# casys-kaist/CoVA

Hardware: AMD Instinct MI355X
Metric: compressed-domain frames/sec (BlobNet+bboxcc) at 1080p b=256 (higher is better)
Workload: dtype f16

## Files before the change

### cova_amd/_lib.py

```python
from __future__ import annotations

import ctypes as C
import os

import numpy as np

_HERE = os.path.dirname(os.path.abspath(__file__))
LIB_PATH = os.path.join(_HERE, "libcovahip.so")

OK = 0
MEM_HOST, MEM_DEVICE = 0, 1
AU_DELTA_UNIT, AU_DISCONT, AU_DROPPABLE = 1, 2, 4


class CovahipError(RuntimeError):
    def __init__(self, status: int, where: str, detail: str = ""):
        self.status = status
        try:
            text = lib().covahip_strerror(status).decode()
        except AttributeError:
            text = "error"
        msg = f"{where}: {text} (status {status})"
        if detail:
            msg += f" [{detail}]"
# ... 142 lines not shown
    "covahip_sort_finalize": (C.c_int, [_P, _P, _SZ, C.POINTER(_SZ), _P, _SZ, C.POINTER(_SZ)]),
    "covahip_sort_mark_seen": (C.c_int, [_P, C.c_uint64]),
    "covahip_sort_num_trackers": (C.c_int, [_P, C.POINTER(_SZ)]),
    "covahip_sort_tracker_info": (C.c_int, [_P, _SZ, C.POINTER(C.c_uint64), C.POINTER(C.c_int),
                                            C.POINTER(C.c_uint64), C.POINTER(C.c_uint64), _P]),
    "covahip_sort_tracker_predict": (C.c_int, [_P, _SZ, C.c_uint64, _P]),
    "covahip_sort_tracker_update": (C.c_int, [_P, _SZ, _P]),
    "covahip_linear_assignment": (_SZ, [_P, _SZ, _SZ, _P, _SZ]),
    "covahip_gopfilter_default_cfg": (None, [C.POINTER(GopFilterCfg)]),
    "covahip_gopfilter_new": (C.c_int, [C.POINTER(GopFilterCfg), C.POINTER(_P)]),
    "covahip_gopfilter_free": (None, [_P]),
    "covahip_gopfilter_push_enc": (C.c_int, [_P, C.c_uint64, C.c_uint64, C.c_uint32]),
    "covahip_gopfilter_push_boxes": (C.c_int, [_P, _P, _SZ, C.c_uint64, _P, _SZ, C.POINTER(_SZ)]),
    "covahip_gopfilter_eos": (C.c_int, [_P, _P, _SZ, C.POINTER(_SZ)]),
    "covahip_gopfilter_take_dropped": (C.c_int, [_P, _P, _SZ, C.POINTER(_SZ)]),
    "covahip_gopfilter_take_track_export": (_SZ, [_P, _P, _SZ, C.POINTER(C.c_int)]),
    "covahip_gopfilter_counters": (C.c_int, [_P, C.POINTER(C.c_uint64), C.POINTER(C.c_uint64),
                                             C.POINTER(C.c_uint64)]),
    "covahip_train_default_cfg": (None, [C.POINTER(TrainCfg)]),
    "covahip_train_create": (C.c_int, [_P, C.POINTER(TrainCfg), _P, _SZ, C.POINTER(_P)]),
    "covahip_train_step": (C.c_int, [_P, _P, _P, C.c_int, C.c_float, C.POINTER(C.c_float), C.c_int]),
    "covahip_train_metrics": (C.c_int, [_P, C.POINTER(C.c_int64)]),
    "covahip_train_weights": (C.c_int, [_P, _P, _SZ, C.POINTER(_SZ)]),
    "covahip_train_grads": (C.c_int, [_P, _P, _SZ]),
    "covahip_train_create_set": (C.c_int, [_P, C.POINTER(TrainCfg), C.c_int, _P, _P, _P, C.POINTER(_P)]),
    "covahip_train_num_models": (C.c_int, [_P, C.POINTER(C.c_int)]),
    "covahip_train_step_set": (C.c_int, [_P, _P, _P, _P, _P, _P, C.c_int]),
    "covahip_train_metrics_m": (C.c_int, [_P, C.c_int, C.POINTER(C.c_int64)]),
    "covahip_train_weights_m": (C.c_int, [_P, C.c_int, _P, _SZ, C.POINTER(_SZ)]),
    "covahip_train_grads_m": (C.c_int, [_P, C.c_int, _P, _SZ]),
    "covahip_train_eval": (C.c_int, [_P, _P, _P, C.c_int, _P, _P, C.POINTER(TrainEvalResult), C.c_int]),
    "covahip_train_eval_set": (C.c_int, [_P, _P, _P, _P, _P, _P, C.POINTER(TrainEvalResult), C.c_int]),
    "covahip_train_state_size": (C.c_int, [_P, C.POINTER(_SZ)]),
    "covahip_train_save_state": (C.c_int, [_P, C.c_uint64, _P, _SZ, C.POINTER(_SZ)]),
    "covahip_train_load_state": (C.c_int, [_P, _P, _SZ, C.POINTER(C.c_uint64)]),
    "covahip_train_destroy": (None, [_P]),
    "covahip_mog_default_cfg": (None, [C.POINTER(MogCfg)]),
    "covahip_mog_create": (C.c_int, [_P, C.POINTER(MogCfg), C.POINTER(_P)]),
    "covahip_mog_apply": (C.c_int, [_P, _P, C.c_int, _P, _P, C.c_int]),
    "covahip_mog_reset": (C.c_int, [_P, C.c_int]),
    "covahip_mog_destroy": (None, [_P]),
}

DEV_PROTOTYPES = {
    "covahip_blobnet_set_impl": (C.c_int, [_P, C.c_int]),
    "covahip_bboxcc_set_wave_cap": (C.c_int, [_P, C.c_int]),
    "covahip_blobnet_set_enc_plan": (C.c_int, [_P, C.c_int, C.c_int, C.c_int]),
    "covahip_dev_clock_mhz": (C.c_int, [_P, C.c_int, C.POINTER(C.c_float)]),
    "covahip_dev_graph_probe": (C.c_int, [_P, _P, C.c_int, _P, C.c_int, C.c_int, _P, _P, C.c_int, _P, C.c_int, C.POINTER(C.c_float),
                                          C.POINTER(C.c_float)]),
    "covahip_dev_bboxcc_overflow": (C.c_int, [_P, C.POINTER(C.c_int32)]),
    "covahip_dev_pipe_queue_plan": (C.c_int, [_P, C.POINTER(C.c_int), C.POINTER(C.c_int)]),
    "covahip_dev_blobnet_buffer": (C.c_int, [_P, C.c_int, C.c_int, C.POINTER(C.c_void_p), C.POINTER(C.c_size_t), C.POINTER(C.c_int32)]),
    "covahip_dev_mog_masks": (C.c_int, [_P, _P, _P, _SZ, C.POINTER(C.c_int)]),
    "covahip_dev_mog_state": (C.c_int, [_P, C.c_int, _P, _P, _P, _P, C.POINTER(C.c_int64)]),
}

_lib = None


def lib() -> C.CDLL:
    global _lib
    if _lib is None:
        san = os.environ.get("COVAHIP_HOST_SAN_LIB")
        if san:
            L = C.CDLL(san)
            for name, (res, args) in list(PROTOTYPES.items()) + list(DEV_PROTOTYPES.items()):
                fn = getattr(L, name, None)
                if fn is not None:
                    fn.restype = res
                    fn.argtypes = args
            _lib = L
            return _lib
        if not os.path.exists(LIB_PATH):
            raise ImportError(
                f"{LIB_PATH} not found: build it with `python -c 'import __graft_entry__ as g; g.build()'` "
                "or `make -C cova_amd/csrc` -- cova_amd has no CPU fallback")
        L = C.CDLL(LIB_PATH)
        for name, (res, args) in list(PROTOTYPES.items()) + list(DEV_PROTOTYPES.items()):
            fn = getattr(L, name)
            fn.restype = res
            fn.argtypes = args
        _lib = L
    return _lib


def check(status: int, where: str, ctx=None) -> None:
    if status != OK:
        detail = ""
        if ctx is not None and status == 3:
            detail = lib().covahip_last_hip_error(ctx).decode()
        raise CovahipError(status, where, detail)
```

### cova_amd/csrc/blobnet.h

```cpp
#pragma once
#include <hip/hip_fp16.h>

#include <vector>

#include "internal.h"

constexpr int BN_T = 4;
constexpr int BN_LEVELS = 4;
constexpr int BN_KTAB_STACKS = 256;

struct BnLevelGeom {
    int H, W;
};

struct BnWorkspace {
    bool ready = false;
    __half *act[BN_LEVELS + 1] = {};
    __half *dact[BN_LEVELS] = {};
    __half *pbuf = nullptr;
    size_t pbuf_frames = 0;
    float *part = nullptr;
    int32_t *d_index = nullptr;
    int32_t *h_index = nullptr;
    size_t index_ints = 0;
    hipEvent_t ev_index = nullptr;
    std::vector<int32_t> last_table;
    int last_n_frames = 0;
    uint8_t *d_models = nullptr;
    uint8_t *h_models = nullptr;
    size_t models_cap = 0;
    hipEvent_t ev_models = nullptr;
    std::vector<uint8_t> last_models;
};

struct covahip_blobnet {
    int H = 0, W = 0, max_batch = 0;
    int n_models = 1;
    BnLevelGeom lv[BN_LEVELS + 1];
    int enc_c[BN_LEVELS + 1] = {3, 16, 32, 64, 128};
    int dec_ci[BN_LEVELS] = {128, 128, 64, 32};
    int dec_co[BN_LEVELS] = {64, 32, 16, 16};
    int dec_cy[BN_LEVELS], dec_cx[BN_LEVELS];
    BnWorkspace ws[COVAHIP_MAX_LANES];
    void *d_prepared = nullptr;
    size_t prepared_bytes = 0;
    struct Prepared *prep = nullptr;
    int fuse_tail = 1;
    int fuse_dec = 1;
    int enc1_tile16 = 1;
    int tail_rows = 1;
    int tail_part = 1;
    int fuse_enc23 = 1;
    int enc_rowtiles = 1;
    int64_t macs_per_frame = 0;
};

constexpr int BN_E1_MAXW = 62;
inline bool bn_level1_on_enc1(const covahip_ctx *ctx, const covahip_blobnet *m) {
    return m->enc1_tile16 && m->enc_c[1] == 16 && m->enc_c[2] == 32 && m->lv[1].W <= BN_E1_MAXW && m->lv[1].H >= 2 &&
           !ctx->enc_plan[1].nbands;
}

int blobnet_prepare_mfma(covahip_ctx *ctx, covahip_blobnet *m, const float *const *h_weights, int n_models);
void blobnet_release_mfma(covahip_ctx *ctx, covahip_blobnet *m);
struct BnCcTail {
    int area_thresh, max_boxes;
    covahip_box *boxes;
    int32_t *counts;
};
struct BnInput {
    const uint8_t *stack = nullptr;
    const uint8_t *frames = nullptr;
    int n_frames = 0;
    const int32_t *index = nullptr;
    const int32_t *h_index = nullptr;
    bool packed = false;
    bool dry = false;
    int model = 0;
    const uint8_t *model_ids = nullptr;
    const uint8_t *frame_models = nullptr;
    bool mixed = false;
};
int blobnet_forward_mfma(covahip_ctx *ctx, covahip_blobnet *m, BnWorkspace &ws, const BnInput &in, int batch, float *d_logits,
                         uint8_t *d_mask, const BnCcTail *cc = nullptr, bool *cc_done = nullptr);
```

### cova_amd/csrc/blobnet.hip

```cpp
#include <algorithm>
#include <cstdlib>
#include <cstring>
#include <vector>

#include "blobnet.h"
#include "covahip_dev.h"

namespace {

constexpr uint32_t W_MAGIC = 0x57485643;
constexpr size_t N_PARAMS = 320305;

}

static void free_model(covahip_ctx *ctx, covahip_blobnet *m) {
    if (!m) return;
    blobnet_release_mfma(ctx, m);
    for (BnWorkspace &ws : m->ws) {
        for (int i = 0; i <= BN_LEVELS; i++)
            if (ws.act[i]) hipFree(ws.act[i]);
        for (int j = 0; j < BN_LEVELS; j++)
            if (ws.dact[j]) hipFree(ws.dact[j]);
        if (ws.pbuf) hipFree(ws.pbuf);
        if (ws.part) hipFree(ws.part);
// ... 270 lines not shown
}

int covahip_blobnet_load_set(covahip_ctx *ctx, int n_models, const void *const *weights, const size_t *weights_bytes, int h_mb,
                             int w_mb, int t, int max_batch) {
    if (!ctx || !weights || !weights_bytes || h_mb <= 0 || w_mb <= 0 || max_batch <= 0) return COVAHIP_ERR_INVALID_ARG;
    if (n_models < 1 || n_models > COVAHIP_MAX_MODELS) return COVAHIP_ERR_INVALID_ARG;
    for (int k = 0; k < n_models; k++)
        if (!weights[k]) return COVAHIP_ERR_INVALID_ARG;
    if (t != BN_T) return COVAHIP_ERR_UNSUPPORTED;
    if (h_mb < 16 || w_mb < 16 || h_mb > 1024 || w_mb > 1024) return COVAHIP_ERR_UNSUPPORTED;
    std::vector<const float *> h_w(n_models);
    bool bad = false;
    for (int k = 0; k < n_models; k++) bad = bad || !(h_w[k] = check_blob(weights[k], weights_bytes[k]));

    COVAHIP_CHECK_HIP(ctx, hipSetDevice(ctx->device));
    covahip_blobnet_destroy(ctx);
    if (bad) return COVAHIP_ERR_BAD_WEIGHTS;
    covahip_blobnet *m = new covahip_blobnet();
    int rc = build_model(ctx, m, h_w.data(), n_models, h_mb, w_mb, max_batch);
    if (rc == COVAHIP_OK && hipStreamSynchronize(ctx->stream) != hipSuccess) rc = COVAHIP_ERR_HIP;
    if (rc) {
        hipStreamSynchronize(ctx->stream);
        (void)hipGetLastError();
        free_model(ctx, m);
        return rc;
    }
    ctx->blobnet = m;
    return COVAHIP_OK;
}

int covahip_blobnet_num_models(covahip_ctx *ctx, int *n_models) {
    if (!ctx || !n_models) return COVAHIP_ERR_INVALID_ARG;
    if (!ctx->blobnet) return COVAHIP_ERR_NOT_LOADED;
    *n_models = ctx->blobnet->n_models;
    return COVAHIP_OK;
}

int covahip_blobnet_macs_per_frame(covahip_ctx *ctx, int64_t *macs) {
    if (!ctx || !macs) return COVAHIP_ERR_INVALID_ARG;
    if (!ctx->blobnet) return COVAHIP_ERR_NOT_LOADED;
    *macs = ctx->blobnet->macs_per_frame;
    return COVAHIP_OK;
}

int covahip_blobnet_set_enc_plan(covahip_ctx *ctx, int level, int nbands, int nbuf) {
    if (!ctx || level < 1 || level > 3 || nbands < 0 || nbands > 64 || (nbands && nbuf != 1 && nbuf != 2)) return COVAHIP_ERR_INVALID_ARG;
    ctx->enc_plan[level].nbands = nbands;
    ctx->enc_plan[level].nbuf = nbands ? nbuf : 0;
    return COVAHIP_OK;
}

int covahip_blobnet_set_impl(covahip_ctx *ctx, int impl) {
    if (!ctx || !ctx->blobnet) return COVAHIP_ERR_NOT_LOADED;
    if (impl != 1 && (impl < 4 || impl > 10)) return COVAHIP_ERR_INVALID_ARG;
    ctx->blobnet->fuse_dec = impl != 4;
    ctx->blobnet->enc1_tile16 = impl != 5;
    ctx->blobnet->enc_rowtiles = impl != 6;
    ctx->blobnet->fuse_enc23 = impl == 7 ? 0 : impl == 8 ? 2 : 1;
    ctx->blobnet->tail_part = impl != 9;
    ctx->blobnet->tail_rows = impl != 10;
    return COVAHIP_OK;
}

static int filter_placed(covahip_ctx *ctx, covahip_blobnet *m, const uint8_t *d_src, int n_frames, const int32_t *stack_index,
                         int batch, int area_thresh, covahip_box *d_boxes, int32_t *d_counts, int max_boxes, float *d_logits,
                         uint8_t *d_mask, bool packed = false, const uint8_t *model_ids = nullptr) {
    if (!d_mask) {
        CtxLane &l = ctx->lane();
        int rc = covahip_ensure_buffer(ctx, &l.cc_scratch, &l.cc_scratch_bytes, (size_t)batch * m->H * m->W);
        if (rc) return rc;
        d_mask = (uint8_t *)l.cc_scratch;
    }
    BnInput in;
    if (n_frames > 0) {
        int rc = prepare_frames(ctx, m, m->ws[ctx->cur_lane], d_src, n_frames, stack_index, batch, in, model_ids);
        if (rc) return rc;
        in.packed = packed;
    } else {
        in.stack = d_src;
    }
    return filter_dev(ctx, in, batch, d_logits, d_mask, true, area_thresh, d_boxes, d_counts, max_boxes, n_frames > 0 ? nullptr : model_ids);
}

static int filter_any(covahip_ctx *ctx, const uint8_t *src, int n_frames, const int32_t *stack_index, int batch,
                      int area_thresh, covahip_box *boxes, int32_t *counts, int max_boxes, float *logits, uint8_t *mask,
                      int mem_kind, const uint8_t *model_ids = nullptr) {
    if (!ctx || batch < 0 || max_boxes < 0 || n_frames < 0) return COVAHIP_ERR_INVALID_ARG;
    covahip_blobnet *m = ctx->blobnet;
    if (!m) return COVAHIP_ERR_NOT_LOADED;
    if (batch == 0) return COVAHIP_OK;
    if (!src || !counts || (!boxes && max_boxes > 0) || batch > m->max_batch) return COVAHIP_ERR_INVALID_ARG;
    if (int rc = check_model_ids(m, model_ids, batch)) return rc;
    COVAHIP_CHECK_HIP(ctx, hipSetDevice(ctx->device));
    const bool by_frames = n_frames > 0;
    const size_t hw = (size_t)m->H * m->W;
    const size_t in_bytes = by_frames ? (size_t)n_frames * hw * 4 : (size_t)batch * BN_T * hw * 4;
    const size_t mask_bytes = (size_t)batch * hw;
    const size_t logit_bytes = mask_bytes * sizeof(float);
    const size_t box_bytes = (size_t)batch * max_boxes * sizeof(covahip_box);
    const size_t cnt_bytes = (size_t)batch * sizeof(int32_t);
    auto al = [](size_t x) { return (x + 255) & ~(size_t)255; };
    if (mem_kind != COVAHIP_MEM_DEVICE && mem_kind != COVAHIP_MEM_HOST) return COVAHIP_ERR_INVALID_ARG;

    if (mem_kind == COVAHIP_MEM_DEVICE) {
        LaneScope lane(ctx);
        if (!lane.ok()) return COVAHIP_ERR_HIP;
        return filter_placed(ctx, m, src, n_frames, stack_index, batch, area_thresh, boxes, counts, max_boxes, logits, mask, false, model_ids);
    }
    if (int rc = covahip_primary_op(ctx)) return rc;
    const uint8_t *d_src = src;
    int rc = covahip_ensure_buffer(ctx, &ctx->stage_in, &ctx->stage_in_bytes, in_bytes);
    if (rc) return rc;
    rc = covahip_ensure_buffer(ctx, &ctx->stage_out, &ctx->stage_out_bytes,
// ... 199 lines not shown
```

### cova_amd/csrc/blobnet_mfma.hip

```cpp
#include <algorithm>
#include <cmath>
#include <cstdlib>
#include <cstring>
#include <mutex>
#include <type_traits>
#include <utility>
#include <vector>

#include "bboxcc_body.h"
#include "bboxcc_wave.h"
#include "blobnet.h"

typedef _Float16 half8 __attribute__((ext_vector_type(8)));
typedef _Float16 half4 __attribute__((ext_vector_type(4)));
typedef float f32x16 __attribute__((ext_vector_type(16)));
typedef float f32x4 __attribute__((ext_vector_type(4)));
typedef _Float16 half2v __attribute__((ext_vector_type(2)));

namespace {

constexpr float BN_EPS = 1e-3f;
constexpr int WG = 256;

struct EncPrep {
// ... 1717 lines not shown
#endif
    dec012_zero_border<128>(t0, p.lv[0], tid);
    dec012_zero_border<128>(t1, p.lv[1], tid);
    dec012_zero_border<64>(t2, p.lv[2], tid);
    for (int b = blockIdx.x; b < p.B; b += gridDim.x) {
        [[maybe_unused]] const uint32_t moff = model_off<MS>(p.model_ids, p.mstride, b);
        if (b != (int)blockIdx.x) lds_barrier();
        PHASE_MARK(0);
        {
            Dec012W<128, 64> w0;
            dec012_load(w0, at_model(p.wf[0], moff), at_model(p.epi[0], moff), wave, lane);
            dec012_stage<0, 128>(t0, p.skip[0] + (size_t)b * p.Ts[0] * p.lv[0].Hi * p.lv[0].Wi * 128, p.lv[0], wave, lane, 0);
            dec012_stage<64, 64>(t1, p.skip[1] + (size_t)b * p.Ts[1] * p.lv[1].Hi * p.lv[1].Wi * 64, p.lv[1], wave, lane, p.lv[0].Hi & 7);
            dec012_stage<32, 32>(t2, p.skip[2] + (size_t)b * p.Ts[2] * p.lv[2].Hi * p.lv[2].Wi * 32, p.lv[2], wave, lane,
                                 (p.lv[0].Hi + p.lv[1].Hi) & 7);
            PHASE_MARK(1);
            wait_vmem();
            lds_barrier();
            PHASE_MARK(2);
            dec012_block<0, 128, 64, 128>(smem, t0, t1, nullptr, nullptr, w0, p.lv[0], p.lv[1], wave, lane);
        }
        PHASE_MARK(3);
        {
            Dec012W<128, 32> w1;
            dec012_load(w1, at_model(p.wf[1], moff), at_model(p.epi[1], moff), wave, lane);
            lds_barrier();
#ifdef PHASE_TIMING
            asm volatile("s_waitcnt vmcnt(0)" ::: "memory");
#endif
            PHASE_MARK(4);
            dec012_block<64, 64, 32, 64>(smem, t1, t2, nullptr, nullptr, w1, p.lv[1], p.lv[2], wave, lane);
        }
        PHASE_MARK(5);
        {
            Dec012W<64, 16> w2;
            dec012_load(w2, at_model(p.wf[2], moff), at_model(p.epi[2], moff), wave, lane);
            lds_barrier();
#ifdef PHASE_TIMING
            asm volatile("s_waitcnt vmcnt(0)" ::: "memory");
#endif
            PHASE_MARK(6);
            dec012_block<32, 32, 16, 0>(smem, t2, nullptr, p.out + (size_t)b * p.lv[2].Hd * p.lv[2].Wd * 16, smem + p.scr_off, w2,
                                        p.lv[2], p.lv[2], wave, lane);
        }
        PHASE_MARK(7);
    }
#ifdef PHASE_TIMING
    if (tid == 0)
        for (int i = 0; i < 9; i++) atomicAdd(&g_phase[48 + i], ph_[i]);
#endif
    WGSPAN_END(3);
}

struct Dec3ccArgs {
    DecArgs d;
    ccbody::CcGeom g;
    ccwave::WvGeom wg;
    int use_wv;
    covahip_box *boxes;
    int32_t *counts;
    int area_thresh, max_boxes;
    int tile_bytes;
    int mfull_off, cc_off;
    int part_off;
    DecMs ms;
};

template <bool WV, bool PART, bool MS = false>
__global__ __launch_bounds__(ccbody::CC_THREADS) void dec3cc_mfma(Dec3ccArgs q) {
    constexpr int C1 = 16, C2 = PART ? 0 : 16, C = C1 + C2, NW = ccbody::CC_THREADS / 64;
    constexpr int KC = C / 16, KSTEPS = 4 * KC, CPP = C / 8, PS = C * 2;
    extern __shared__ __attribute__((aligned(16))) uint8_t smem[];
    const DecArgs &p = q.d;
    const int tid = threadIdx.x, lane = tid & 63, wave = tid >> 6;
    const int TC = p.Wi + 2;
    const int GW = p.Wi + 1, GH = p.Hi + 1;
    const int kh = lane >> 5;
    float fbias = p.epi[0];
    uint8_t *const mfull = smem + q.mfull_off;
    WGSPAN_BEGIN();
#ifdef PHASE_TIMING
    unsigned long long ph_[9] = {0, 0, 0, 0, 0, 0, 0, 0, 0}, last_ = __builtin_amdgcn_s_memrealtime();
#endif

    for (int b = blockIdx.x; b < p.B; b += gridDim.x) {
        half8 wf[KSTEPS];
        if constexpr (MS) {
            const uint32_t moff = model_off<MS>(q.ms.model_ids, q.ms.mstride, b);
            fbias = at_model(p.epi, moff)[0];
#pragma unroll
            for (int ks = 0; ks < KSTEPS; ks++) wf[ks] = at_model(p.wfrag, moff)[ks * 64 + lane];
        } else {
#pragma unroll
            for (int ks = 0; ks < KSTEPS; ks++) wf[ks] = p.wfrag[ks * 64 + lane];
        }
        auto stage = [&](int band, uint8_t *buf) {
            const int u0 = band * GH / p.nbands, u1 = (band + 1) * GH / p.nbands;
            const int RC = TC * CPP;
            const int nchunk = (u1 - u0 + 1) * RC;
            const __half *su = p.up + ((size_t)b) * p.Hi * p.Wi * C1;
            const __half *ss = p.skip + ((size_t)b * p.Ts) * p.Hi * p.Wi * C2;
            for (int s0 = wave * 64; s0 < nchunk; s0 += NW * 64) {
                const int sidx = s0 + lane;
                if (sidx < nchunk) {
                    const int r = fdiv(sidx, p.mRC), within = sidx - r * RC;
                    const int c = within / CPP, chp = within % CPP;
                    const int cb = (chp ^ swz_eval<CPP>(p.swz, c, r)) * 8;
                    const int y = u0 - 1 + r, x = c - 1;
                    const void *src = p.zero;
                    if (y >= 0 && y < p.Hi && x >= 0 && x < p.Wi) {
                        const size_t pix = (size_t)y * p.Wi + x;
                        src = (PART || cb < C1) ? (const void *)(su + pix * C1 + cb) : (const void *)(ss + pix * C2 + (cb - C1));
                    }
                    glds16(src, buf + s0 * 16);
                }
            }
        };
// ... 33 lines not shown
                        const int s = swz_eval<CPP>(p.swz, xx, yy);
#pragma unroll
                        for (int kc = 0; kc < KC; kc++) {
                            const half8 av = *reinterpret_cast<const half8 *>(cur + pbase + (((kc * 2 + kh) ^ s) * 16));
                            acc = __builtin_amdgcn_mfma_f32_32x32x16_f16(wf[(a * 2 + bb) * KC + kc], av, acc, 0, 0, 0);
                        }
                    }
                if (qi < npos && kh == 0) {
                    const int u = u0 + ul;
                    f32x4 pl = {0.f, 0.f, 0.f, 0.f};
                    if constexpr (PART) pl = reinterpret_cast<const f32x4 *>(smem + q.part_off)[u * GW + v];
#pragma unroll
                    for (int r = 0; r < 4; r++) {
                        const int Y = 2 * u + (r >> 1) - p.cy, X = 2 * v + (r & 1) - p.cx;
                        if (Y >= 0 && Y < p.Hd && X >= 0 && X < p.Wd) {
                            float l = acc[r] + fbias;
                            if constexpr (PART) l += pl[r];
                            if (p.logits) p.logits[((size_t)b * p.Hd + Y) * p.Wd + X] = l;
                            mfull[Y * p.Wd + X] = l > 0.f ? 1 : 0;
                        }
                    }
                }
            }
        }
        PHASE_MARK(4);
        lds_barrier();
        PHASE_MARK(5);
        if (p.mask) {
            uint8_t *dst = p.mask + (size_t)b * p.Hd * p.Wd;
            const int nbytes = p.Hd * p.Wd;
            if ((nbytes & 3) == 0 && (reinterpret_cast<uintptr_t>(p.mask) & 3) == 0) {
                for (int i = tid; i < nbytes / 4; i += NW * 64)
                    reinterpret_cast<uint32_t *>(dst)[i] = reinterpret_cast<const uint32_t *>(mfull)[i];
            } else {
                for (int i = tid; i < nbytes; i += NW * 64) dst[i] = mfull[i];
            }
        }
        PHASE_MARK(6);
        if constexpr (WV)
            ccwave::frame_wg<ccbody::CC_THREADS>(mfull, smem + q.cc_off, q.wg, q.area_thresh, q.boxes + (size_t)b * q.max_boxes,
                                                 q.counts + b, q.max_boxes, tid);
        else
            ccbody::bboxcc_frame(mfull, smem + q.cc_off, q.g, q.area_thresh, q.boxes + (size_t)b * q.max_boxes, q.counts + b,
                                 q.max_boxes, tid);
        PHASE_MARK(7);
    }
#ifdef PHASE_TIMING
    if (tid == 0)
        for (int i = 0; i < 9; i++) atomicAdd(&g_phase[64 + i], ph_[i]);
#endif
    WGSPAN_END(4);
}

template <bool MS = false>
__global__ __launch_bounds__(ccbody::CC_THREADS) void dec3cc_rows_mfma(Dec3ccArgs q) {
    constexpr int NW = ccbody::CC_THREADS / 64, PS = 32;
    extern __shared__ __attribute__((aligned(16))) uint8_t smem[];
    const DecArgs &p = q.d;
    const int tid = threadIdx.x, lane = tid & 63, wave = tid >> 6;
    const int TC = p.Wi + 2, GW = p.Wi + 1, GH = p.Hi + 1;
    const int kh = lane >> 5, pos = lane & 31;
    const float fbias0 = p.epi[0];
    uint32_t *const planes = reinterpret_cast<uint32_t *>(smem + q.mfull_off);
    const f32x4 *const part = reinterpret_cast<const f32x4 *>(smem + q.part_off);
    WGSPAN_BEGIN();
#ifdef PHASE_TIMING
    unsigned long long ph_[9] = {0, 0, 0, 0, 0, 0, 0, 0, 0}, last_ = __builtin_amdgcn_s_memrealtime();
#endif
    uint32_t lc[2][2];
#pragma unroll
    for (int h = 0; h < 2; h++)
#pragma unroll
        for (int bb = 0; bb < 2; bb++) {
            const int xx = min(32 * h + pos, GW - 1) + 1 - bb;
            lc[h][bb] = (uint32_t)(xx * PS + ((kh ^ ((xx >> 3) & 1)) << 4));
        }
    const int row_b = TC * PS;
    for (int b = blockIdx.x; b < p.B; b += gridDim.x) {
        const uint32_t moff = model_off<MS>(q.ms.model_ids, q.ms.mstride, b);
        const float fbias = MS ? at_model(p.epi, moff)[0] : fbias0;
        half8 wf[4];
#pragma unroll
        for (int ks = 0; ks < 4; ks++) wf[ks] = (MS ? at_model(p.wfrag, moff) : p.wfrag)[ks * 64 + lane];
        if (b != (int)blockIdx.x) lds_barrier();
        PHASE_MARK(0);
        {
            const uint8_t *ps = reinterpret_cast<const uint8_t *>(p.part) + (size_t)b * GH * GW * 16;
            const int nch = GH * GW;
            for (int s0 = wave * 64; s0 < nch; s0 += NW * 64)
                if (s0 + lane < nch) glds16(ps + (size_t)(s0 + lane) * 16, smem + q.part_off + s0 * 16);
        }
        {
            const __half *su = p.up + (size_t)b * p.Hi * p.Wi * 16;
            const int NI = 2 * p.Wi;
            for (int y = wave; y < p.Hi; y += NW) {
                const __half *rowp = su + (size_t)y * p.Wi * 16;
                uint8_t *rowl = smem + ((y + 1) * TC + 1) * PS;
                for (int q0 = 0; q0 < NI; q0 += 64) {
                    const int qq = q0 + lane, px = qq >> 1;
                    const int cb = ((qq & 1) ^ (((px + 1) >> 3) & 1)) * 8;
                    if (qq < NI) glds16(rowp + px * 16 + cb, rowl + q0 * 16);
                }
            }
            const int n_rows = 4 * TC, n_cols = 4 * p.Hi;
            for (int i = tid; i < n_rows + n_cols; i += NW * 64) {
                int piece;
                if (i < n_rows) {
                    piece = i < 2 * TC ? i : (p.Hi + 1) * 2 * TC + (i - 2 * TC);
                } else {
                    const int j = i - n_rows, y = j >> 2, k = j & 3;
                    piece = (y + 1) * 2 * TC + (k < 2 ? k : (p.Wi + 1) * 2 + (k - 2));
                }
                *reinterpret_cast<uint4 *>(smem + piece * 16) = uint4{0, 0, 0, 0};
            }
            for (int i = tid; i < q.wg.rows_bytes / 4; i += NW * 64) planes[i] = 0;
        }
        PHASE_MARK(1);
        wait_vmem();
        lds_barrier();
        PHASE_MARK(2);
        for (int t = wave; t < 2 * GH; t += NW) {
            const int u = t >> 1, h = t & 1;
            if (32 * h >= GW) continue;
            const uint32_t rb = (uint32_t)(u * row_b);
            const uint32_t a00 = rb + row_b + (h ? lc[1][0] : lc[0][0]), a01 = rb + row_b + (h ? lc[1][1] : lc[0][1]);
            const uint32_t a10 = rb + (h ? lc[1][0] : lc[0][0]), a11 = rb + (h ? lc[1][1] : lc[0][1]);
            f32x16 acc;
#pragma unroll
            for (int r = 0; r < 16; r++) acc[r] = 0.f;
            acc = __builtin_amdgcn_mfma_f32_32x32x16_f16(wf[0], *reinterpret_cast<const half8 *>(smem + a00), acc, 0, 0, 0);
            acc = __builtin_amdgcn_mfma_f32_32x32x16_f16(wf[1], *reinterpret_cast<const half8 *>(smem + a01), acc, 0, 0, 0);
            acc = __builtin_amdgcn_mfma_f32_32x32x16_f16(wf[2], *reinterpret_cast<const half8 *>(smem + a10), acc, 0, 0, 0);
            acc = __builtin_amdgcn_mfma_f32_32x32x16_f16(wf[3], *reinterpret_cast<const half8 *>(smem + a11), acc, 0, 0, 0);
            const int v = 32 * h + pos;
            const bool live = kh == 0 && v < GW;
            const f32x4 pl = part[u * GW + min(v, GW - 1)];
            float l[4];
#pragma unroll
            for (int r = 0; r < 4; r++) l[r] = (acc[r] + fbias) + pl[r];
            if (p.logits && live) {
#pragma unroll
                for (int r = 0; r < 4; r++) {
                    const int Y = 2 * u + (r >> 1) - p.cy, X = 2 * v + (r & 1) - p.cx;
                    if (Y >= 0 && Y < p.Hd && X >= 0 && X < p.Wd) p.logits[((size_t)b * p.Hd + Y) * p.Wd + X] = l[r];
                }
            }
#pragma unroll
            for (int r = 0; r < 4; r++) {
                const uint64_t bits = (uint64_t)(uint32_t)__ballot(live && l[r] > 0.f) << (32 * h);
                const int Y = 2 * u + (r >> 1) - p.cy, X0 = (r & 1) - p.cx;
                const int pln = X0 & 1, sh = X0 >> 1;
                const int nb = (p.Wd - pln + 1) >> 1;
                uint64_t w = sh >= 0 ? bits << sh : bits >> (-sh);
                w &= nb >= 64 ? ~0ull : ((1ull << nb) - 1);
                if (Y >= 0 && Y < p.Hd && lane == 0) {
                    uint32_t *rw = planes + (Y + 1) * 4 + 2 * pln;
                    if ((uint32_t)w) atomicOr(rw, (uint32_t)w);
                    if ((uint32_t)(w >> 32)) atomicOr(rw + 1, (uint32_t)(w >> 32));
                }
            }
        }
        PHASE_MARK(4);
        lds_barrier();
        PHASE_MARK(5);
        if (p.mask) {
            uint32_t *dst = reinterpret_cast<uint32_t *>(p.mask + (size_t)b * p.Hd * p.Wd);
            const int wq = p.Wd >> 2, nq = p.Hd * wq;
            for (int i = tid; i < nq; i += NW * 64) {
                const int y = fdiv(i, p.mRC), xq = i - y * wq;
                const int bx = 2 * xq;
                const uint32_t *rw = planes + (y + 1) * 4 + (bx >> 5);
                const uint32_t e2 = (rw[0] >> (bx & 31)) & 3u, o2 = (rw[2] >> (bx & 31)) & 3u;
                dst[i] = (e2 & 1u) | ((o2 & 1u) << 8) | ((e2 >> 1) << 16) | ((o2 >> 1) << 24);
            }
        }
        PHASE_MARK(6);
        ccwave::frame_wg<ccbody::CC_THREADS, true>(nullptr, smem + q.cc_off, q.wg, q.area_thresh, q.boxes + (size_t)b * q.max_boxes,
                                                   q.counts + b, q.max_boxes, tid, planes);
        PHASE_MARK(7);
    }
#ifdef PHASE_TIMING
    if (tid == 0)
        for (int i = 0; i < 9; i++) atomicAdd(&g_phase[64 + i], ph_[i]);
#endif
    WGSPAN_END(4);
}

void enc_epilogue(int cout, bool allpos, const float *bias, const float *gamma, const float *beta, const float *mean,
                  const float *var, std::vector<float> &wscale, float *epi) {
    wscale.assign(cout, 1.f);
    for (int c = 0; c < cout; c++) {
        const float sc = gamma[c] / std::sqrt(var[c] + BN_EPS), sh = beta[c] - mean[c] * sc;
        wscale[c] = sc;
        const float bp = bias[c] * sc;
        epi[cout + c] = bp + sh;
        if (allpos) {
            epi[c] = -bp;
            epi[2 * cout + c] = 0.f;
        } else {
            epi[c] = sc >= 0.f ? -bp : -3.0e38f;
            epi[2 * cout + c] = sc >= 0.f ? 3.0e38f : -bp;
        }
    }
}

void prep_enc0(bool allpos, const float *k, const float *bias, const float *gamma, const float *beta, const float *mean,
               const float *var, const float *w1, const float *w2, _Float16 *wfrag, float *epi) {
    std::vector<float> ws;
    enc_epilogue(16, allpos, bias, gamma, beta, mean, var, ws, epi);
    for (int set = 0; set < 2; set++)
        for (int ks = 0; ks < 2; ks++)
            for (int l = 0; l < 64; l++)
                for (int j = 0; j < 8; j++) {
                    const int n = l & 15, g = l >> 4;
                    const int px = 2 * (g & 1) + (j >> 2), ch = j & 3;
                    const int kx = set == 0 ? px - 1 : px;
                    int ky = -1;
                    if (ks == 0) ky = g >> 1;
                    else if ((g >> 1) == 0) ky = 2;
                    float w = 0.f;
                    if (ky >= 0 && kx >= 0 && kx < 3 && ch < 3) w = k[((ky * 3 + kx) * 3 + ch) * 16 + n] * ws[n] / 6.0f;
                    wfrag[((set * 2 + ks) * 64 + l) * 8 + j] = f2h(w);
                }
    std::memcpy(epi + 48, w1, 16 * sizeof(float));
    std::memcpy(epi + 64, w2, 16 * sizeof(float));
}

// ... 658 lines not shown
            return launch(f, "dec2_mfma", dec_mfma<32, 32, 16, false, MS.value>, p.grid, 256, p.lds, p.a, p.am);
        }, f.ms));
    return launched(f, with_bools([&](auto HALF, auto MS) {
        return launch(f, "dec3_final_mfma", dec_mfma<16, HALF.value ? 0 : 16, 16, true, MS.value>, p.grid, 256, p.lds, p.a, p.am);
    }, p.half, f.ms));
}
int run_dec_block(const Fwd &f, int j) {
    DecPlan p;
    if (int rc = plan_dec_block(f, j, p)) return rc;
    return launch_dec_block(f, j, p);
}

bool run_tail_fused(const Fwd &f, const DecPlan &p) {
    const BnLevelGeom in = p.in, out = p.out;
    const int GH = p.GH;
    Dec3ccArgs t;
    size_t cc_bytes = ccbody::cc_plan(out.H, out.W, t.g);
    t.use_wv = f.ctx->cc_wave_cap >= 0 && ccwave::wv_plan(out.H, out.W, ((out.H + 1) / 2) * ((out.W + 1) / 2), t.wg) ? 1 : 0;
    if (t.use_wv) cc_bytes = (size_t)t.wg.wave_bytes;
    if (!cc_bytes) return false;
    const size_t mfull = ((size_t)out.H * out.W + 15) & ~(size_t)15;
    const size_t partb = p.half ? (size_t)GH * (in.W + 1) * 16 : 0;
    int best_nb = 0;
    long long best_cost = -1;
    for (int nb = 1; nb <= GH; nb++) {
        const size_t tb = (((size_t)((GH + nb - 1) / nb) + 1) * p.row_bytes + 15) & ~(size_t)15;
        const size_t nbuf = nb == 1 ? 1 : 2;
        if (std::max(nbuf * tb, cc_bytes) + mfull + partb > 160 * 1024 - 512) continue;
        long long rounds = 0;
        for (int k = 0; k < nb; k++) {
            const int nu = (k + 1) * GH / nb - k * GH / nb;
            rounds += ((nu * (in.W + 1) + 31) / 32 + 15) / 16;
        }
        const long long cost = rounds * 8 + nb;
        if (best_cost < 0 || cost < best_cost) { best_cost = cost; best_nb = nb; }
    }
    if (!best_nb) return false;
    const size_t tb = (((size_t)((GH + best_nb - 1) / best_nb) + 1) * p.row_bytes + 15) & ~(size_t)15;
    t.d = p.a;
    t.ms = p.am;
    t.d.nbands = best_nb; t.d.mNb = magic(best_nb);
    t.d.swz = choose_swz(false, p.ci, in.W, 0, (GH + best_nb - 1) / best_nb);
    t.boxes = f.cc->boxes; t.counts = f.cc->counts;
    t.area_thresh = f.cc->area_thresh; t.max_boxes = f.cc->max_boxes;
    t.tile_bytes = (int)tb; t.cc_off = 0;
    t.mfull_off = (int)std::max((best_nb == 1 ? 1 : 2) * tb, cc_bytes);
    t.part_off = (int)((size_t)t.mfull_off + mfull);
    const size_t tl = (size_t)t.part_off + partb;
    const int grid = std::min(f.batch, 2 * f.num_cu);
    if (p.half && t.use_wv && best_nb == 1 && in.W + 1 <= 64 && f.m->tail_rows && (out.W & 7) == 0 &&
        (size_t)t.wg.rows_bytes <= mfull && (!f.d_mask || (reinterpret_cast<uintptr_t>(f.d_mask) & 3) == 0)) {
        t.d.swz = Swz{3, 1, 0, 0, 0};
        t.d.mRC = magic(out.W / 4);
        return !with_bools([&](auto MS) {
            return launch(f, "dec3_bboxcc_fused", dec3cc_rows_mfma<MS.value>, grid, ccbody::CC_THREADS, tl, t);
        }, f.ms);
    }
    return !with_bools([&](auto WV, auto PART, auto MS) {
        return launch(f, "dec3_bboxcc_fused", dec3cc_mfma<WV.value, PART.value, MS.value>, grid, ccbody::CC_THREADS, tl, t);
    }, t.use_wv != 0, p.half, f.ms);
}

}

int blobnet_forward_mfma(covahip_ctx *ctx, covahip_blobnet *m, BnWorkspace &ws, const BnInput &inp, int batch, float *d_logits,
                         uint8_t *d_mask, const BnCcTail *cc, bool *cc_done) {
    if (cc_done) *cc_done = false;
    const Prepared *pr = m->prep;
    const bool dry = inp.dry;
    const bool by_frames = inp.frames != nullptr || (dry && inp.n_frames > 0);
    const bool ms = inp.model_ids != nullptr || (dry && inp.mixed);
    Fwd f{ctx, m, pr, ws, inp, batch,
          (const uint8_t *)m->d_prepared + (ms ? 0 : (size_t)inp.model * pr->total), (uint32_t)pr->total,
          ms, dry, by_frames, ctx->props.multiProcessorCount,
          by_frames ? inp.frames : inp.stack, by_frames ? inp.n_frames : batch * BN_T, by_frames ? inp.index : nullptr,
          d_logits, d_mask, cc};
    if ((size_t)f.n_frames > ws.pbuf_frames && !dry) return COVAHIP_ERR_INVALID_ARG;

    int rc = run_enc0p(f);
    if (rc) return rc;
    if (!run_enc1_tile16(f, rc)) rc = run_enc_level(f, 1);
    if (rc) return rc;
    if (!run_enc23(f, rc)) {
        rc = run_enc_level(f, 2);
        if (!rc) rc = run_enc_level(f, 3);
    }
    if (rc) return rc;
    if (!run_dec012(f, rc))
        for (int j = 0; j < BN_LEVELS - 1 && !rc; j++) rc = run_dec_block(f, j);
    if (rc) return rc;
    DecPlan last;
    rc = plan_dec_block(f, BN_LEVELS - 1, last);
    if (rc) return rc;
    if (!(cc && m->fuse_tail && run_tail_fused(f, last))) return launch_dec_block(f, BN_LEVELS - 1, last);
    if (cc_done) *cc_done = true;
    return launched(f, COVAHIP_OK);
}

#if defined(PHASE_TIMING) || defined(WGSPAN_ONLY)
extern "C" int covahip_dev_wgspan_read(unsigned long long *out, int kid) {
    return hipMemcpyFromSymbol(out, HIP_SYMBOL(g_wgspan), sizeof(unsigned long long) * 1024 * 4, sizeof(unsigned long long) * 1024 * 4 * kid) != hipSuccess;
}
#endif
#ifdef WGSPAN_ONLY
extern "C" int covahip_dev_itemspan_read(unsigned long long *out, int kid) {
    return hipMemcpyFromSymbol(out, HIP_SYMBOL(g_itemspan), sizeof(unsigned long long) * 1024 * 16, sizeof(unsigned long long) * 1024 * 16 * kid) != hipSuccess;
}
#endif
#ifdef PHASE_TIMING
extern "C" int covahip_dev_ccphase_read(unsigned long long *out8, int reset) {
    if (hipMemcpyFromSymbol(out8, HIP_SYMBOL(g_ccph), sizeof(g_ccph)) != hipSuccess) return 1;
    if (reset) {
        unsigned long long z[8] = {0};
        if (hipMemcpyToSymbol(HIP_SYMBOL(g_ccph), z, sizeof(z)) != hipSuccess) return 1;
    }
    return 0;
}
extern "C" int covahip_dev_phase_read(unsigned long long *out64, int reset) {
    if (hipMemcpyFromSymbol(out64, HIP_SYMBOL(g_phase), sizeof(g_phase)) != hipSuccess) return 1;
    if (reset) {
        unsigned long long z[80] = {0};
        if (hipMemcpyToSymbol(HIP_SYMBOL(g_phase), z, sizeof(z)) != hipSuccess) return 1;
    }
    return 0;
}
#endif
```

### cova_amd/elements.py

```python
from __future__ import annotations

import ctypes as C

import numpy as np

from . import _lib as L
from . import weights as W

FLOW_OK = "ok"
FLOW_DROPPED = "dropped"


def _ptr(a: np.ndarray) -> int:
    return a.ctypes.data


def _optr(a: np.ndarray | None) -> int | None:
    return None if a is None else a.ctypes.data


class Context:

    def __init__(self, device_id: int = 0):
        self._lib = L.lib()
# ... 88 lines not shown
        ow, oh = self.transform_caps(width, height)
        out_size = ow * oh * 4
        self.size_per_buf = out_size // self.timestep
        self.out_size = out_size
        self.stop()
        h = C.c_void_p()
        L.check(self._lib.covahip_stack_new(self.size_per_buf, self.timestep, self.gamma, C.byref(h)), "stack_new")
        self._h = h
        return ow, oh

    def transform(self, inbuf: bytes | np.ndarray):
        a = np.frombuffer(inbuf, dtype=np.uint8) if not isinstance(inbuf, np.ndarray) else inbuf.reshape(-1)
        a = np.ascontiguousarray(a, dtype=np.uint8)
        out = np.empty(self.out_size, dtype=np.uint8)
        em = C.c_int()
        L.check(self._lib.covahip_stack_push(self._h, _ptr(a), a.size, _ptr(out), out.size, C.byref(em)), "stack_push")
        return (FLOW_OK, out) if em.value else (FLOW_DROPPED, None)

    def stop(self):
        if self._h:
            self._lib.covahip_stack_free(self._h)
            self._h = None

    __del__ = stop


class BlobNetInfer:

    def __init__(self, ctx: Context, weights_flat, h_mb: int, w_mb: int, max_batch: int,
                 timestep: int = 4):
        self.ctx, self.h, self.w, self.t, self.max_batch = ctx, h_mb, w_mb, timestep, max_batch
        self._lib = L.lib()
        if isinstance(weights_flat, (list, tuple)):
            blobs = [W.to_bytes(w) for w in weights_flat]
            ptrs = (C.c_char_p * max(1, len(blobs)))(*blobs)
            sizes = (C.c_size_t * max(1, len(blobs)))(*[len(b) for b in blobs])
            L.check(self._lib.covahip_blobnet_load_set(ctx.handle, len(blobs), ptrs, sizes, h_mb, w_mb, timestep, max_batch),
                    "covahip_blobnet_load_set", ctx.handle)
        else:
            blob = W.to_bytes(weights_flat)
            L.check(self._lib.covahip_blobnet_load(ctx.handle, blob, len(blob), h_mb, w_mb, timestep, max_batch),
                    "covahip_blobnet_load", ctx.handle)

    @property
    def num_models(self) -> int:
        v = C.c_int()
        L.check(self._lib.covahip_blobnet_num_models(self.ctx.handle, C.byref(v)), "covahip_blobnet_num_models")
        return v.value

    def set_enc_plan(self, level: int, nbands: int, nbuf: int = 1):
        L.check(self._lib.covahip_blobnet_set_enc_plan(self.ctx.handle, level, nbands, nbuf), "covahip_blobnet_set_enc_plan")

    def set_impl(self, impl: str):
        L.check(self._lib.covahip_blobnet_set_impl(self.ctx.handle, {"mfma": 1, "dec_separate": 4, "enc1_legacy": 5, "enc_general_tiles": 6, "enc23_separate": 7, "enc23_force": 8, "tail_skip_tensor": 9, "tail_band_tiles": 10}[impl]), "set_impl")

    def read_buffer(self, which: int, index: int = 0) -> np.ndarray:
        p, n, dims = C.c_void_p(), C.c_size_t(), (C.c_int32 * 5)()
        L.check(self._lib.covahip_dev_blobnet_buffer(self.ctx.handle, which, index, C.byref(p), C.byref(n), dims),
                "covahip_dev_blobnet_buffer", self.ctx.handle)
        out = np.empty(tuple(d for d in dims if d), dtype=np.float32 if which == 3 else np.float16)
        assert p.value and out.nbytes == n.value, (which, index, n.value, tuple(dims))
        self.ctx.d2h(out, p.value)
        return out

    @property
    def macs_per_frame(self) -> int:
        v = C.c_int64()
        L.check(self._lib.covahip_blobnet_macs_per_frame(self.ctx.handle, C.byref(v)), "macs_per_frame")
        return v.value

    def infer(self, stack: np.ndarray, want_logits: bool = True, model_ids=None):
        stack = np.ascontiguousarray(stack, dtype=np.uint8)
        b = stack.shape[0]
        assert stack.shape == (b, self.t * self.h, self.w, 4), stack.shape
        logits = np.empty((b, self.h, self.w), dtype=np.float32) if want_logits else None
        mask = np.empty((b, self.h, self.w), dtype=np.uint8)
        ids = _ids(model_ids, b)
        L.check(self._lib.covahip_blobnet_forward_m(self.ctx.handle, _ptr(stack), _optr(ids), b, _ptr(logits) if want_logits else None,
                                                    _ptr(mask), L.MEM_HOST), "covahip_blobnet_forward_m", self.ctx.handle)
        return logits, mask

    def infer_device(self, d_stack: int, batch: int, d_logits: int | None, d_mask: int | None, model_ids=None):
        ids = _ids(model_ids, batch)
        L.check(self._lib.covahip_blobnet_forward_m(self.ctx.handle, d_stack, _optr(ids), batch, d_logits, d_mask, L.MEM_DEVICE),
                "covahip_blobnet_forward_m", self.ctx.handle)

    def filter(self, stack: np.ndarray, cc_threshold: int, max_boxes: int = 256, want_mask: bool = False, model_ids=None):
        return self.filter_full(stack, cc_threshold, max_boxes, want_mask, False, model_ids)[:3]

    def filter_full(self, stack: np.ndarray, cc_threshold: int, max_boxes: int = 256, want_mask: bool = False,
                    want_logits: bool = False, model_ids=None):
        stack = np.ascontiguousarray(stack, dtype=np.uint8)
        b = stack.shape[0]
        boxes = np.zeros((b, max_boxes), dtype=L.BOX_DTYPE)
        counts = np.zeros(b, dtype=np.int32)
        mask = np.empty((b, self.h, self.w), dtype=np.uint8) if want_mask else None
        logits = np.empty((b, self.h, self.w), dtype=np.float32) if want_logits else None
        ids = _ids(model_ids, b)
        L.check(self._lib.covahip_filter_forward_m(self.ctx.handle, _ptr(stack), _optr(ids), b, cc_threshold, _ptr(boxes), _ptr(counts),
                                                   max_boxes, _ptr(logits) if want_logits else None, _ptr(mask) if want_mask else None,
                                                   L.MEM_HOST),
                "covahip_filter_forward_m", self.ctx.handle)
        return boxes, counts, mask, logits

    def filter_frames(self, frames: np.ndarray, stack_index: np.ndarray | None, cc_threshold: int, max_boxes: int = 256,
                      want_mask: bool = False, want_logits: bool = False, model_ids=None):
        frames = np.ascontiguousarray(frames, dtype=np.uint8)
# ... 465 lines not shown
```

### include/covahip_dev.h

```cpp
#ifndef COVAHIP_DEV_H
#define COVAHIP_DEV_H

#include "covahip.h"

#ifdef __cplusplus
extern "C" {
#endif

int covahip_blobnet_set_impl(covahip_ctx *ctx, int impl);

int covahip_bboxcc_set_wave_cap(covahip_ctx *ctx, int cap);
int covahip_dev_bboxcc_overflow(covahip_ctx *ctx, int32_t *out4);

int covahip_blobnet_set_enc_plan(covahip_ctx *ctx, int level, int nbands, int nbuf);

int covahip_dev_blobnet_buffer(covahip_ctx *ctx, int which, int index, void **dptr, size_t *bytes, int32_t dims[5]);

int covahip_dev_clock_mhz(covahip_ctx *ctx, int busy_us, float *mhz);

int covahip_dev_graph_probe(covahip_ctx *ctx, const uint8_t *d_frames, int n_frames, const int32_t *stack_index, int batch,
                            int area_thresh, covahip_box *d_boxes, int32_t *d_counts, int max_boxes, uint8_t *d_mask, int iters,
                            float *ms_direct, float *ms_graph);

struct covahip_pipe;
int covahip_dev_pipe_queue_plan(struct covahip_pipe *pipe, int *lanes_on_upload_queue, int *lanes_on_result_queue);

struct covahip_mog;
int covahip_dev_mog_masks(struct covahip_mog *m, uint8_t *raw, uint8_t *filled, size_t cap, int *n_frames);
int covahip_dev_mog_state(struct covahip_mog *m, int stream, float *W, float *V, float *M, uint8_t *nmodes, int64_t *n);

#ifdef __cplusplus
}
#endif
#endif
```

Before: 2.443 million.

## Pipeline fused dec3+bboxcc tail loads in row bands through registers

Adds a banded variant of the fused dec3/bboxcc kernel. It splits the input rows into 3 or 4 bands and prefetches each band's activation rows and partial sums into registers one band ahead. MFMA tiles for a band start as soon as that band lands in LDS, instead of waiting for the whole frame to load. A host-side planner picks the band count by default and falls back to the original single-pass path when the geometry does not fit. The cost is extra barriers per band and higher register pressure from the staged loads.

```diff
diff --git a/cova_amd/_lib.py b/cova_amd/_lib.py
--- a/cova_amd/_lib.py
+++ b/cova_amd/_lib.py
@@ -218,6 +218,7 @@
     "covahip_dev_bboxcc_overflow": (C.c_int, [_P, C.POINTER(C.c_int32)]),
     "covahip_dev_pipe_queue_plan": (C.c_int, [_P, C.POINTER(C.c_int), C.POINTER(C.c_int)]),
     "covahip_dev_blobnet_buffer": (C.c_int, [_P, C.c_int, C.c_int, C.POINTER(C.c_void_p), C.POINTER(C.c_size_t), C.POINTER(C.c_int32)]),
+    "covahip_dev_tail_band_plan": (C.c_int, [C.c_int, C.c_int, C.c_int, C.c_int, C.c_int, C.c_int, C.POINTER(C.c_int), _P, _P]),
     "covahip_dev_mog_masks": (C.c_int, [_P, _P, _P, _SZ, C.POINTER(C.c_int)]),
     "covahip_dev_mog_state": (C.c_int, [_P, C.c_int, _P, _P, _P, _P, C.POINTER(C.c_int64)]),
 }
diff --git a/cova_amd/csrc/blobnet.h b/cova_amd/csrc/blobnet.h
--- a/cova_amd/csrc/blobnet.h
+++ b/cova_amd/csrc/blobnet.h
@@ -49,6 +49,7 @@
     int fuse_dec = 1;
     int enc1_tile16 = 1;
     int tail_rows = 1;
+    int tail_bands = 0;
     int tail_part = 1;
     int fuse_enc23 = 1;
     int enc_rowtiles = 1;
diff --git a/cova_amd/csrc/blobnet.hip b/cova_amd/csrc/blobnet.hip
--- a/cova_amd/csrc/blobnet.hip
+++ b/cova_amd/csrc/blobnet.hip
@@ -346,13 +346,14 @@
 
 int covahip_blobnet_set_impl(covahip_ctx *ctx, int impl) {
     if (!ctx || !ctx->blobnet) return COVAHIP_ERR_NOT_LOADED;
-    if (impl != 1 && (impl < 4 || impl > 10)) return COVAHIP_ERR_INVALID_ARG;
+    if (impl != 1 && (impl < 4 || impl > 12)) return COVAHIP_ERR_INVALID_ARG;
     ctx->blobnet->fuse_dec = impl != 4;
     ctx->blobnet->enc1_tile16 = impl != 5;
     ctx->blobnet->enc_rowtiles = impl != 6;
     ctx->blobnet->fuse_enc23 = impl == 7 ? 0 : impl == 8 ? 2 : 1;
     ctx->blobnet->tail_part = impl != 9;
     ctx->blobnet->tail_rows = impl != 10;
+    ctx->blobnet->tail_bands = impl == 11 ? 1 : impl == 12 ? 4 : 0;
     return COVAHIP_OK;
 }
 
diff --git a/cova_amd/csrc/blobnet_mfma.hip b/cova_amd/csrc/blobnet_mfma.hip
--- a/cova_amd/csrc/blobnet_mfma.hip
+++ b/cova_amd/csrc/blobnet_mfma.hip
@@ -1793,6 +1793,26 @@
     WGSPAN_END(3);
 }
 
+constexpr int TAIL_MAXB = 4;
+struct TailBands {
+    int nb;
+    int row_end[TAIL_MAXB], mask_end[TAIL_MAXB];
+};
+int tail_band_plan(int Hi, int Wi, int Hd, int cy, int nw, int want, TailBands &tb) {
+    const int tiles_per_row = Wi + 1 > 32 ? 2 : 1;
+    int nb = want > 0 ? want : 3;
+    if (want <= 0 && (Hi < 2 * nw || (Hi / nb) * tiles_per_row < nw)) nb = 1;
+    const int rows = nb > 0 ? (Hi + nb - 1) / nb : Hi;
+    if ((nb != 3 && nb != 4) || nb > Hi || rows > nw || (rows + 1) * (Wi + 1) > 64 * nw) nb = 1;
+    tb.nb = nb;
+    for (int k = 0; k < TAIL_MAXB; k++) {
+        const int e = k < nb ? (int)((long long)(k + 1) * Hi / nb) : Hi;
+        tb.row_end[k] = e;
+        tb.mask_end[k] = k >= nb - 1 ? Hd : std::max(0, std::min(Hd, 2 * e - cy));
+    }
+    return nb;
+}
+
 struct Dec3ccArgs {
     DecArgs d;
     ccbody::CcGeom g;
@@ -1804,6 +1824,7 @@
     int tile_bytes;
     int mfull_off, cc_off;
     int part_off;
+    TailBands tb;
     DecMs ms;
 };
 
@@ -1943,7 +1964,7 @@
     WGSPAN_END(4);
 }
 
-template <bool MS = false>
+template <bool MS = false, int NB = 0>
 __global__ __launch_bounds__(ccbody::CC_THREADS) void dec3cc_rows_mfma(Dec3ccArgs q) {
     constexpr int NW = ccbody::CC_THREADS / 64, PS = 32;
     extern __shared__ __attribute__((aligned(16))) uint8_t smem[];
@@ -1953,7 +1974,7 @@
     const int kh = lane >> 5, pos = lane & 31;
     const float fbias0 = p.epi[0];
     uint32_t *const planes = reinterpret_cast<uint32_t *>(smem + q.mfull_off);
-    const f32x4 *const part = reinterpret_cast<const f32x4 *>(smem + q.part_off);
+    [[maybe_unused]] const f32x4 *const part = reinterpret_cast<const f32x4 *>(smem + q.part_off);
     WGSPAN_BEGIN();
 #ifdef PHASE_TIMING
     unsigned long long ph_[9] = {0, 0, 0, 0, 0, 0, 0, 0, 0}, last_ = __builtin_amdgcn_s_memrealtime();
@@ -1967,6 +1988,7 @@
             lc[h][bb] = (uint32_t)(xx * PS + ((kh ^ ((xx >> 3) & 1)) << 4));
         }
     const int row_b = TC * PS;
+    const int NI = 2 * p.Wi;
     for (int b = blockIdx.x; b < p.B; b += gridDim.x) {
         const uint32_t moff = model_off<MS>(q.ms.model_ids, q.ms.mstride, b);
         const float fbias = MS ? at_model(p.epi, moff)[0] : fbias0;
@@ -1975,24 +1997,8 @@
         for (int ks = 0; ks < 4; ks++) wf[ks] = (MS ? at_model(p.wfrag, moff) : p.wfrag)[ks * 64 + lane];
         if (b != (int)blockIdx.x) lds_barrier();
         PHASE_MARK(0);
-        {
-            const uint8_t *ps = reinterpret_cast<const uint8_t *>(p.part) + (size_t)b * GH * GW * 16;
-            const int nch = GH * GW;
-            for (int s0 = wave * 64; s0 < nch; s0 += NW * 64)
-                if (s0 + lane < nch) glds16(ps + (size_t)(s0 + lane) * 16, smem + q.part_off + s0 * 16);
-        }
-        {
-            const __half *su = p.up + (size_t)b * p.Hi * p.Wi * 16;
-            const int NI = 2 * p.Wi;
-            for (int y = wave; y < p.Hi; y += NW) {
-                const __half *rowp = su + (size_t)y * p.Wi * 16;
-                uint8_t *rowl = smem + ((y + 1) * TC + 1) * PS;
-                for (int q0 = 0; q0 < NI; q0 += 64) {
-                    const int qq = q0 + lane, px = qq >> 1;
-                    const int cb = ((qq & 1) ^ (((px + 1) >> 3) & 1)) * 8;
-                    if (qq < NI) glds16(rowp + px * 16 + cb, rowl + q0 * 16);
-                }
-            }
+        const __half *su = p.up + (size_t)b * p.Hi * p.Wi * 16;
+        auto zero_border_and_planes = [&]() {
             const int n_rows = 4 * TC, n_cols = 4 * p.Hi;
             for (int i = tid; i < n_rows + n_cols; i += NW * 64) {
                 int piece;
@@ -2005,14 +2011,8 @@
                 *reinterpret_cast<uint4 *>(smem + piece * 16) = uint4{0, 0, 0, 0};
             }
             for (int i = tid; i < q.wg.rows_bytes / 4; i += NW * 64) planes[i] = 0;
-        }
-        PHASE_MARK(1);
-        wait_vmem();
-        lds_barrier();
-        PHASE_MARK(2);
-        for (int t = wave; t < 2 * GH; t += NW) {
-            const int u = t >> 1, h = t & 1;
-            if (32 * h >= GW) continue;
+        };
+        auto tile = [&](int u, int h, auto get_pl) {
             const uint32_t rb = (uint32_t)(u * row_b);
             const uint32_t a00 = rb + row_b + (h ? lc[1][0] : lc[0][0]), a01 = rb + row_b + (h ? lc[1][1] : lc[0][1]);
             const uint32_t a10 = rb + (h ? lc[1][0] : lc[0][0]), a11 = rb + (h ? lc[1][1] : lc[0][1]);
@@ -2025,7 +2025,7 @@
             acc = __builtin_amdgcn_mfma_f32_32x32x16_f16(wf[3], *reinterpret_cast<const half8 *>(smem + a11), acc, 0, 0, 0);
             const int v = 32 * h + pos;
             const bool live = kh == 0 && v < GW;
-            const f32x4 pl = part[u * GW + min(v, GW - 1)];
+            const f32x4 pl = get_pl(v);
             float l[4];
 #pragma unroll
             for (int r = 0; r < 4; r++) l[r] = (acc[r] + fbias) + pl[r];
@@ -2050,20 +2050,101 @@
                     if ((uint32_t)(w >> 32)) atomicOr(rw + 1, (uint32_t)(w >> 32));
                 }
             }
-        }
-        PHASE_MARK(4);
-        lds_barrier();
-        PHASE_MARK(5);
-        if (p.mask) {
+        };
+        auto mask_out = [&](int y0, int y1) {
             uint32_t *dst = reinterpret_cast<uint32_t *>(p.mask + (size_t)b * p.Hd * p.Wd);
-            const int wq = p.Wd >> 2, nq = p.Hd * wq;
-            for (int i = tid; i < nq; i += NW * 64) {
+            const int wq = p.Wd >> 2;
+            for (int i = y0 * wq + tid; i < y1 * wq; i += NW * 64) {
                 const int y = fdiv(i, p.mRC), xq = i - y * wq;
                 const int bx = 2 * xq;
                 const uint32_t *rw = planes + (y + 1) * 4 + (bx >> 5);
                 const uint32_t e2 = (rw[0] >> (bx & 31)) & 3u, o2 = (rw[2] >> (bx & 31)) & 3u;
                 dst[i] = (e2 & 1u) | ((o2 & 1u) << 8) | ((e2 >> 1) << 16) | ((o2 >> 1) << 24);
             }
+        };
+        if constexpr (NB == 0) {
+            {
+                const uint8_t *ps = reinterpret_cast<const uint8_t *>(p.part) + (size_t)b * GH * GW * 16;
+                const int nch = GH * GW;
+                for (int s0 = wave * 64; s0 < nch; s0 += NW * 64)
+                    if (s0 + lane < nch) glds16(ps + (size_t)(s0 + lane) * 16, smem + q.part_off + s0 * 16);
+            }
+            for (int y = wave; y < p.Hi; y += NW) {
+                const __half *rowp = su + (size_t)y * p.Wi * 16;
+                uint8_t *rowl = smem + ((y + 1) * TC + 1) * PS;
+                for (int q0 = 0; q0 < NI; q0 += 64) {
+                    const int qq = q0 + lane, px = qq >> 1;
+                    const int cb = ((qq & 1) ^ (((px + 1) >> 3) & 1)) * 8;
+                    if (qq < NI) glds16(rowp + px * 16 + cb, rowl + q0 * 16);
+                }
+            }
+            zero_border_and_planes();
+            PHASE_MARK(1);
+            wait_vmem();
+            lds_barrier();
+            PHASE_MARK(2);
+            for (int t = wave; t < 2 * GH; t += NW) {
+                const int u = t >> 1, h = t & 1;
+                if (32 * h >= GW) continue;
+                tile(u, h, [&](int v) { return part[u * GW + min(v, GW - 1)]; });
+            }
+            PHASE_MARK(4);
+            lds_barrier();
+            PHASE_MARK(5);
+            if (p.mask) mask_out(0, p.Hd);
+        } else {
+            const f32x4 *pg = reinterpret_cast<const f32x4 *>(p.part) + (size_t)b * GH * GW;
+            f32x4 *const partw = reinterpret_cast<f32x4 *>(smem + q.part_off);
+            const int wv = __builtin_amdgcn_readfirstlane(wave);
+            uint32_t roff[2];
+#pragma unroll
+            for (int c = 0; c < 2; c++) {
+                const int qq = min(64 * c + lane, NI - 1), px = qq >> 1;
+                roff[c] = (uint32_t)(px * 16 + ((qq & 1) ^ (((px + 1) >> 3) & 1)) * 8);
+            }
+            uint4 ra0, ra1, rb0, rb1;
+            f32x4 pa, pb;
+            auto band_g0 = [&](int k) { return k ? q.tb.row_end[k - 1] : 0; };
+            auto band_g1 = [&](int k) { return k == NB - 1 ? GH : q.tb.row_end[k]; };
+            auto request = [&](int k, uint4 &r0, uint4 &r1, f32x4 &pv) {
+                const int y = band_g0(k) + wv;
+                const __half *rowp = su + (size_t)y * p.Wi * 16;
+                const bool mine = y < q.tb.row_end[k];
+                r0 = *reinterpret_cast<const uint4 *>(mine ? rowp + roff[0] : su);
+                r1 = *reinterpret_cast<const uint4 *>(mine ? rowp + roff[1] : su);
+                pv = pg[band_g0(k) * GW + min(tid, (band_g1(k) - band_g0(k)) * GW - 1)];
+            };
+            request(0, ra0, ra1, pa);
+            request(1, rb0, rb1, pb);
+            zero_border_and_planes();
+            PHASE_MARK(1);
+            int t = wave;
+            auto band = [&](int k, uint4 &r0, uint4 &r1, f32x4 &pv) {
+                const int g0 = band_g0(k), g1 = band_g1(k);
+                if (g0 + wv < q.tb.row_end[k]) {
+                    uint8_t *rowl = smem + ((g0 + wv + 1) * TC + 1) * PS;
+                    *reinterpret_cast<uint4 *>(rowl + lane * 16) = r0;
+                    if (64 + lane < NI) *reinterpret_cast<uint4 *>(rowl + (64 + lane) * 16) = r1;
+                }
+                partw[g0 * GW + min(tid, (g1 - g0) * GW - 1)] = pv;
+                if (k + 2 < NB) request(k + 2, r0, r1, pv);
+                lds_barrier();
+                PHASE_MARK(k ? 3 : 2);
+                for (; t < 2 * g1; t += NW) {
+                    const int u = t >> 1, h = t & 1;
+                    if (32 * h >= GW) continue;
+                    tile(u, h, [&](int v) { return part[u * GW + min(v, GW - 1)]; });
+                }
+            };
+            band(0, ra0, ra1, pa);
+            band(1, rb0, rb1, pb);
+            band(2, ra0, ra1, pa);
+            if constexpr (NB > 3) band(3, rb0, rb1, pb);
+            static_assert(NB == 3 || NB == 4, "the bands are written out");
+            PHASE_MARK(4);
+            lds_barrier();
+            PHASE_MARK(5);
+            if (p.mask) mask_out(0, p.Hd);
         }
         PHASE_MARK(6);
         ccwave::frame_wg<ccbody::CC_THREADS, true>(nullptr, smem + q.cc_off, q.wg, q.area_thresh, q.boxes + (size_t)b * q.max_boxes,
@@ -2828,8 +2909,17 @@
         (size_t)t.wg.rows_bytes <= mfull && (!f.d_mask || (reinterpret_cast<uintptr_t>(f.d_mask) & 3) == 0)) {
         t.d.swz = Swz{3, 1, 0, 0, 0};
         t.d.mRC = magic(out.W / 4);
+        const int nb = tail_band_plan(in.H, in.W, out.H, t.d.cy, ccbody::CC_THREADS / 64, f.m->tail_bands, t.tb);
+        if (nb == 3)
+            return !with_bools([&](auto MS) {
+                return launch(f, "dec3_bboxcc_fused", dec3cc_rows_mfma<MS.value, 3>, grid, ccbody::CC_THREADS, tl, t);
+            }, f.ms);
+        if (nb == 4)
+            return !with_bools([&](auto MS) {
+                return launch(f, "dec3_bboxcc_fused", dec3cc_rows_mfma<MS.value, 4>, grid, ccbody::CC_THREADS, tl, t);
+            }, f.ms);
         return !with_bools([&](auto MS) {
-            return launch(f, "dec3_bboxcc_fused", dec3cc_rows_mfma<MS.value>, grid, ccbody::CC_THREADS, tl, t);
+            return launch(f, "dec3_bboxcc_fused", dec3cc_rows_mfma<MS.value, 0>, grid, ccbody::CC_THREADS, tl, t);
         }, f.ms);
     }
     return !with_bools([&](auto WV, auto PART, auto MS) {
@@ -2873,6 +2963,20 @@
     return launched(f, COVAHIP_OK);
 }
 
+extern "C" int covahip_dev_tail_band_plan(int hi, int wi, int hd, int cy, int waves, int want, int *n_bands, int32_t *row_end,
+                                          int32_t *mask_end) {
+    if (hi < 1 || wi < 1 || hd < 1 || cy < 0 || cy > 1 || waves < 1 || want < 0 || !n_bands || !row_end || !mask_end)
+        return COVAHIP_ERR_INVALID_ARG;
+    TailBands tb;
+    const int nb = tail_band_plan(hi, wi, hd, cy, waves, want, tb);
+    for (int k = 0; k < nb; k++) {
+        row_end[k] = tb.row_end[k];
+        mask_end[k] = tb.mask_end[k];
+    }
+    *n_bands = nb;
+    return COVAHIP_OK;
+}
+
 #if defined(PHASE_TIMING) || defined(WGSPAN_ONLY)
 extern "C" int covahip_dev_wgspan_read(unsigned long long *out, int kid) {
     return hipMemcpyFromSymbol(out, HIP_SYMBOL(g_wgspan), sizeof(unsigned long long) * 1024 * 4, sizeof(unsigned long long) * 1024 * 4 * kid) != hipSuccess;
diff --git a/cova_amd/elements.py b/cova_amd/elements.py
--- a/cova_amd/elements.py
+++ b/cova_amd/elements.py
@@ -164,7 +164,7 @@
         L.check(self._lib.covahip_blobnet_set_enc_plan(self.ctx.handle, level, nbands, nbuf), "covahip_blobnet_set_enc_plan")
 
     def set_impl(self, impl: str):
-        L.check(self._lib.covahip_blobnet_set_impl(self.ctx.handle, {"mfma": 1, "dec_separate": 4, "enc1_legacy": 5, "enc_general_tiles": 6, "enc23_separate": 7, "enc23_force": 8, "tail_skip_tensor": 9, "tail_band_tiles": 10}[impl]), "set_impl")
+        L.check(self._lib.covahip_blobnet_set_impl(self.ctx.handle, {"mfma": 1, "dec_separate": 4, "enc1_legacy": 5, "enc_general_tiles": 6, "enc23_separate": 7, "enc23_force": 8, "tail_skip_tensor": 9, "tail_band_tiles": 10, "tail_one_band": 11, "tail_four_bands": 12}[impl]), "set_impl")
 
     def read_buffer(self, which: int, index: int = 0) -> np.ndarray:
         p, n, dims = C.c_void_p(), C.c_size_t(), (C.c_int32 * 5)()
diff --git a/include/covahip_dev.h b/include/covahip_dev.h
--- a/include/covahip_dev.h
+++ b/include/covahip_dev.h
@@ -22,6 +22,8 @@
                             int area_thresh, covahip_box *d_boxes, int32_t *d_counts, int max_boxes, uint8_t *d_mask, int iters,
                             float *ms_direct, float *ms_graph);
 
+int covahip_dev_tail_band_plan(int hi, int wi, int hd, int cy, int waves, int want, int *n_bands, int32_t *row_end, int32_t *mask_end);
+
 struct covahip_pipe;
 int covahip_dev_pipe_queue_plan(struct covahip_pipe *pipe, int *lanes_on_upload_queue, int *lanes_on_result_queue);
 
```

Result: slower. 2.409 million (-1.4%).
